# swiss-territorial-data-lab/proj-roadsurf

Hardware: AMD Instinct MI355X
Metric: tiles_per_sec_512x512x3 (higher is better)
Workload: dtype f16 hi + lo operand planes (22 significand bits, 3 MFMA products per product) / f32 accumulate; 1 GPU; Mask R-CNN R50-FPN inference, batch 16 of 512x512 3-band tiles per GPU (BASELINE configs[1]), 800x800 network input; seeded synthetic weights, saturated: 1000 proposals and 100 detections per tile; batch_per_gpu=16, lanes=2, lane_streams=independent, num_classes=2, weights=random

## Files before the change

include/rs_engine.h:

```cpp
#ifndef RS_ENGINE_H
#define RS_ENGINE_H

#include <stddef.h>
#include <stdint.h>

#ifdef __cplusplus
extern "C" {
#endif

#define RS_ABI_VERSION 1
#define RS_SPEC_MAX_LEVELS 5
#define RS_SPEC_MAX_ANCHORS 8
#define RS_NUM_PHASES 3
#define RS_MASK_SIDE 28

typedef struct rs_spec {
  int32_t struct_size;
  int32_t in_channels;
  int32_t flip_channels;
  float pixel_mean[4];
  float pixel_std[4];
  int32_t min_size_test;
  int32_t max_size_test;
  int32_t size_divisibility;
// ... 75 lines not shown
int rs_engine_set_profiling(rs_engine* e, int mode);
int rs_engine_stage_count(rs_engine* e);
int rs_engine_stage_info(rs_engine* e, int i, char* name_out, double* ms_total, int* calls, double* flops, double* bytes);
int rs_engine_saturation(rs_engine* e, int64_t* counts, int cap);
int rs_engine_stage_kernel(rs_engine* e, int i, char* name_out);
int rs_engine_stage_variant(rs_engine* e, int i);

int rs_engine_tensor(rs_engine* e, const char* name, void** dev_ptr, int* dtype, int* ndim, int64_t dims[5], int* halo);
int rs_engine_tensor_count(rs_engine* e);
int rs_engine_tensor_name(rs_engine* e, int i, char* name_out );

int rs_engine_net_shape(rs_engine* e, int* resized_h, int* resized_w, int* padded_h, int* padded_w);


int rs_op_conv2d(const void* in, const void* w, const float* bias, void* out, const void* residual,
                 const void* upsample_add, int n, int hi, int wi, int cin, int in_halo, int kh, int kw,
                 int stride, int pad, int cout, int kpad, int out_halo, int relu, int out_f32, int deconv2x,
                 int variant, int use_glds, void* stream);

int rs_op_bneck_tail(const void* t1, const void* w2, const float* b2, const void* w3p, const float* b3, const void* x, void* out,
                     const void* w1p, const float* b1, void* t1n, const void* x0, const void* wsc, int n, int h, int w, int width,
                     void* stream);

int rs_op_bneck_tail_split(const void* t1, int64_t t1_lo, const void* w2, const float* s2, const float* b2, const void* w3p, const float* s3,
                           const float* b3, const void* x, int64_t x_lo, void* out, int64_t out_lo, const void* w1p, const float* s1,
                           const float* b1, void* t1n, int64_t t1n_lo, const void* x0, int64_t x0_lo, int n, int h, int w, int width,
                           void* stream);

int rs_op_mask_overlap(const uint8_t* det_masks, int n_det, const uint8_t* label_masks, int n_labels, int h, int w, int32_t* inter,
                       int32_t* label_area, void* stream);
int rs_engine_label_overlap(rs_engine* e, int tile, const uint8_t* label_masks_dev, int n_labels, int32_t* inter_dev, int32_t* label_area_dev);

int rs_op_conv_variant(int m, int cin, int k, int cout, int cin2, int deconv2x, int out_f32, int* stages_out);

int rs_debug_set_conv_probe(void* buffer);

int rs_op_set_saturation_counter(void* dev_u64);

int rs_op_conv2d_split(const void* in, int64_t in_lo, const void* w, int64_t w_lo, const float* wscale, const float* bias, void* out, int64_t out_lo,
                       const void* residual, int64_t res_lo, const void* upsample_add, int64_t up_lo,
                       int n, int hi, int wi, int cin, int in_halo, int kh, int kw, int stride, int pad, int cout, int kpad,
                       int out_halo, int relu, int out_f32, int deconv2x, int variant, void* stream);

int rs_op_conv2d_dual(const void* in, const void* in2, const void* w, const float* bias, void* out,
                      int n, int hi, int wi, int cin, int in_halo, int kh, int kw, int stride, int pad,
                      int h2, int w2, int cin2, int in2_halo, int stride2,
                      int cout, int kpad, int out_halo, int relu, int variant, void* stream);

int rs_op_conv2d_dgrad(const void* dy, const void* w_t, void* dx, const void* res, const float* res32, const void* mask,
                       const void* down, int n, int hi, int wi, int cin, int ho, int wo, int cout, int kh, int kw, int stride,
                       int pad, int kpad, int halo, int variant, void* stream);

int rs_op_conv2d_wgrad(const void* dy, const void* in, float* grad, const float* scale, int n, int hi, int wi, int cin,
                       int in_halo, int kh, int kw, int stride, int pad, int cout, int kpad, int dy_halo, int splits,
                       void* stream);
int rs_op_conv2d_wgrad_f32(const void* dy, const void* in, float* grad, const float* scale, int n, int hi, int wi, int cin,
                       int in_halo, int kh, int kw, int stride, int pad, int cout, int kpad, int dy_halo, int splits,
                       void* stream);

int rs_op_nms(const float* boxes, const int32_t* counts, const uint8_t* valid, uint8_t* keep,
              int segments, int cap, float thresh, void* stream);

int rs_op_roi_align(const void* const feats[4], const int32_t heights[4], const int32_t widths[4],
                    const float scales[4], int nlevels, const float* rois, int n_rois, int rois_per_image,
                    int P, int out_halo, void* out, int32_t* levels_out, void* stream);

// ... 90 lines not shown
```

proj_roadsurf_amd/csrc/common.h:

```cpp
#pragma once
#include <hip/hip_runtime.h>
#include <stdint.h>
#include <stdio.h>

typedef _Float16 half_t;
typedef _Float16 half4 __attribute__((ext_vector_type(4)));
typedef _Float16 half8 __attribute__((ext_vector_type(8)));
typedef float f32x4 __attribute__((ext_vector_type(4)));

#define RS_OK 0
#define RS_ERR_ARG -1
#define RS_ERR_HIP -2
#define RS_ERR_BLOB -3
#define RS_ERR_UNSUPPORTED -4

void rs_set_error(const char* fmt, ...);

#define RS_HIP(expr)                                                                       \
  do {                                                                                     \
    hipError_t _e = (expr);                                                                \
    if (_e != hipSuccess) {                                                                \
      rs_set_error("%s:%d: %s -> %s", __FILE__, __LINE__, #expr, hipGetErrorString(_e));   \
      return RS_ERR_HIP;                                                                   \
    }                                                                                      \
// ... 220 lines not shown
int wgrad_splits(const WgradParams& p);
int launch_conv_wgrad(const WgradParams& p, hipStream_t stream);

struct PreprocParams {
  const uint8_t* tiles;
  half_t* out;
  const int* hb;
  const int* hk;
  const int* vb;
  const int* vk;
  int N, H, W, C;
  int new_h, new_w;
  int out_Hp, out_Wp;
  int ksh, ksv;
  int need_h, need_v;
  int flip;
  int out_f32;
  long long out_lo;
  float mean[4], stdv[4];
  unsigned long long* sat;
};
int launch_preprocess(const PreprocParams& p, hipStream_t s);
int launch_maxpool(const half_t* in, half_t* out, int N, int Hi, int Wi, int Ho, int Wo, int C, hipStream_t s);
int launch_subsample2(const half_t* in, half_t* out, int N, int Hi, int Wi, int Ho, int Wo, int C, hipStream_t s);
int launch_maxpool_f32(const float* in, float* out, int N, int Hi, int Wi, int Ho, int Wo, int C, hipStream_t s);
int launch_maxpool_split(const half_t* in, long long in_lo, half_t* out, long long out_lo, int N, int Hi, int Wi, int Ho, int Wo, int C, hipStream_t s);
int launch_subsample2_split(const half_t* in, long long in_lo, half_t* out, long long out_lo, int N, int Hi, int Wi, int Ho, int Wo, int C, hipStream_t s);
int launch_subsample2_f32(const float* in, float* out, int N, int Hi, int Wi, int Ho, int Wo, int C, hipStream_t s);
int launch_conv_f32(const ConvParams& p, hipStream_t stream, int force_valu = 0, int tile = 0);
int launch_conv_deep(const ConvParams& p, hipStream_t stream, int tile_px = 256);
int rs_device_cu_count();
bool conv_wreg_ok(const ConvParams& p);
int launch_conv_wreg(const ConvParams& p, hipStream_t stream, int waves = 0);
int launch_conv_deep_multi(const ConvParams& common, const ConvSeg* segs, const int* m_per_image, int nseg, int images, hipStream_t stream);
```

proj_roadsurf_amd/csrc/conv_igemm.hip:

```cpp
#include "common.h"

namespace {

template <int WPX, int WCH, int MI, int NJ>
struct Tile {
  static constexpr int NW = WPX * WCH;
  static constexpr int NT = NW * 64;
  static constexpr int BM = WPX * NJ * 16;
  static constexpr int BN = WCH * MI * 16;
  static constexpr int STAGE = (BM + BN) * 128;
  static constexpr int LDS = 2 * STAGE + 1024;
};

__device__ __forceinline__ void glds16(const half_t* g, char* lds_wave_base) {
  __builtin_amdgcn_global_load_lds((const __attribute__((address_space(1))) void*)g,
                                   (__attribute__((address_space(3))) void*)lds_wave_base, 16, 0, 0);
}

template <int WPX, int WCH, int MI, int NJ, bool SMALLC, bool GLDS, bool PERSIST, bool TRAIN = false, bool SPLIT = false>
__global__ __launch_bounds__(WPX* WCH * 64) void conv_igemm_kernel(const ConvParams p) {
  using T = Tile<WPX, WCH, MI, NJ>;
  constexpr int NW = T::NW, BM = T::BM, BN = T::BN;
  constexpr int PA = BM / (NW * 8);
  constexpr int PW = (BN + NW * 8 - 1) / (NW * 8);
// ... 465 lines not shown
  const void* k;
  if (p.split) {
    RS_CHECK(use_glds > 0 && !train && p.wscale, RS_ERR_UNSUPPORTED, "conv: the split-operand mode needs LDS-DMA staging, the row scales and no training epilogue");
    k = (const void*)conv_igemm_kernel<WPX, WCH, MI, NJ, SMALLC, true, false, false, true>;
  } else if (train) {
    RS_CHECK(use_glds && !SMALLC, RS_ERR_UNSUPPORTED, "conv: training epilogue options need LDS-DMA staging and Cin >= 64");
    if constexpr (!SMALLC) k = (const void*)conv_igemm_kernel<WPX, WCH, MI, NJ, false, true, false, true>;
    else k = nullptr;
  } else if constexpr (CAN_PERSIST) {
    k = persistent ? (const void*)conv_igemm_kernel<WPX, WCH, MI, NJ, SMALLC, true, true>
                   : (use_glds ? (const void*)conv_igemm_kernel<WPX, WCH, MI, NJ, SMALLC, true, false>
                               : (const void*)conv_igemm_kernel<WPX, WCH, MI, NJ, SMALLC, false, false>);
  } else {
    k = use_glds ? (const void*)conv_igemm_kernel<WPX, WCH, MI, NJ, SMALLC, true, false>
                 : (const void*)conv_igemm_kernel<WPX, WCH, MI, NJ, SMALLC, false, false>;
  }
  static bool attr[5] = {false, false, false, false, false};
  const int ai = p.split ? 4 : (train ? 3 : (persistent ? 2 : (use_glds ? 1 : 0)));
  if (!attr[ai]) {
    RS_HIP(hipFuncSetAttribute(k, hipFuncAttributeMaxDynamicSharedMemorySize, T::LDS));
    attr[ai] = true;
  }
  const unsigned grid = (persistent && !p.split) ? 256u * (unsigned)bpc : (unsigned)nblk;
  ConvParams pc = p;
  void* args[] = {&pc};
  RS_HIP(hipLaunchKernel(k, dim3(grid), dim3(T::NT), args, lds, stream));
  return RS_OK;
}

}

thread_local int g_last_conv_variant = -2;

int conv_choose_variant(ConvParams& p, int force_variant, int use_glds) {
  const RsDebug& D = rs_debug();
  const int nk2 = p.in2 ? (p.Cin2 >> 6) : 0;
  const bool smallc = p.Cin < 64;
  const int nk = (p.split ? 3 : 1) * (smallc ? (p.Kpad >> 6) : p.KH * p.KW * (p.Cin >> 6) + nk2);
  if (p.stages == 0) {
    const bool shallow = nk <= D.conv_single_stage_nk;
    if (D.conv_persist >= 1 && shallow && p.mode != 2 && !p.split) { p.stages = 2; p.persist = 2; }
    else { p.stages = shallow ? 1 : 2; p.persist = D.conv_persist >= 2 && p.mode != 2 ? -1 : 0; }
  }
  if (force_variant >= 0) return force_variant;
  const int rows = p.Cout * (p.mode != 0 ? 4 : 1);
  const int nkd = smallc ? 0 : nk;
  const long long tiles0 = (long long)cdiv(p.M, 128) * (rows / 128 > 0 ? rows / 128 : 1);
  const long long tiles4 = (long long)cdiv(p.M, 256) * (rows / 256 > 0 ? rows / 256 : 1);
  if (rows <= 16) return 2;
  if (!D.conv_tuned || p.mode != 0 || smallc) return rows % 128 == 0 ? 0 : 1;
  if (rows % 128 != 0) return 8;
  if (rows % 256 == 0 && nkd >= 8 && D.conv_deep && D.deep_tile_px && use_glds > 0 && !p.in2 && !p.m_count && !p.down && !p.res32 && !p.mask && p.out_stride <= 1) {
    const int ncu = 256;
    auto cost = [&](int nj) {
      const long long t = (long long)cdiv(p.M, 32 * nj) * (rows / 256);
      const long long r = t % ncu;
      const double rounds = (double)(t / ncu) + (r == 0 ? 0.0 : (nj == 8 && D.deep_tail && 2 * r <= ncu ? 0.75 : 1.0));
      return rounds * (nj + 15);
    };
    int best = 8;
    double cb = cost(8);
    for (int nj = 7; nj >= 5; --nj) {
      const long long t = (long long)cdiv(p.M, 32 * nj) * (rows / 256);
      if (4 * t >= 3 * ncu && cost(nj) < 0.95 * cb && cost(nj) < (best == 8 ? 1e30 : cost(best))) best = nj;
    }
    if (best != 8) return 10 + best;
  }
  if (p.split && rows % 256 == 0 && nkd >= 8 && tiles4 >= 64 && tiles4 < 240 && D.conv_deep && use_glds > 0 && !p.in2 && p.out_stride <= 1) return 12;
  if (p.in2 && rows % 256 == 0 && nkd >= 6) return tiles4 >= 600 ? 4 : (tiles0 < 1250 ? 7 : 0);
  if (rows % 256 == 0 && nkd >= 8 && tiles4 >= 240)
    return (D.conv_deep && use_glds > 0 && !p.in2 && p.out_stride <= 1) ? 12 : 4;
  if (D.conv_wreg && !p.split && use_glds > 0 && conv_wreg_ok(p) && (long long)cdiv(p.M, 32) * (p.Cout >> 8) * 5 >= 48ll * rs_device_cu_count()) return 22;
  if (rows % 256 == 0 && nkd <= 4 && p.M >= 40000) return D.conv_wide_px == 64 ? 10 : 14;
  if (nkd <= 4 || tiles0 < 1250) return 7;
  return 0;
}

int launch_conv(const ConvParams& p_in, hipStream_t stream, int force_variant, int use_glds) {
  if (use_glds < 0) {
    RS_CHECK(!p_in.in2, RS_ERR_UNSUPPORTED, "conv: the fp32 kernel has no second K source");
    g_last_conv_variant = -1;
    return launch_conv_f32(p_in, stream, use_glds == -2, force_variant);
  }
  ConvParams p = p_in;
  const int nk2 = p.in2 ? (p.Cin2 >> 6) : 0;
  const bool train_opts = p.down || p.res32 || p.mask || p.out_stride > 1;
  RS_CHECK(p.M > 0, RS_ERR_ARG, "conv: M=%d", p.M);
  RS_CHECK(p.Kpad % 64 == 0, RS_ERR_ARG, "conv: Kpad %d not a multiple of 64", p.Kpad);
  const bool smallc = p.Cin < 64;
  if (smallc) {
    RS_CHECK((p.Cin == 8 || p.Cin == 4) && p.koff != nullptr, RS_ERR_ARG, "conv: small-Cin path needs Cin 4 or 8 and a koff table");
  } else {
    RS_CHECK(p.Cin % 64 == 0, RS_ERR_ARG, "conv: Cin %d not a multiple of 64", p.Cin);
    RS_CHECK(p.KH * p.KW * p.Cin + nk2 * 64 <= p.Kpad, RS_ERR_ARG, "conv: K exceeds Kpad");
  }
  if (p.in2) RS_CHECK(!smallc && p.mode == 0 && p.Cin2 % 64 == 0 && p.Cin2 > 0 && p.stride2 >= 1, RS_ERR_ARG, "conv: bad second K source (Cin2 %d)", p.Cin2);
  const int rows = p.Cout * (p.mode != 0 ? 4 : 1);
  int v = conv_choose_variant(p, force_variant, use_glds);
  if (v == 22 && p.mode == 2 && !conv_wreg_ok(p)) v = 14;
  RS_CHECK(!(train_opts && (p.mode != 0 || (v == 12 && p.out_stride > 1) || (v >= 15 && v <= 20))), RS_ERR_UNSUPPORTED, "conv: training epilogue options need mode 0 (and no scatter on conv_deep)");
  if (v == 22 || v == 23 || v == 25 || v == 26) {
    RS_CHECK(conv_wreg_ok(p) && !train_opts, RS_ERR_UNSUPPORTED, "conv: variant %d takes 1x1 / Cin 256 / Cout %% 256 == 0 inference layers only", v);
    g_last_conv_variant = v;
    return launch_conv_wreg(p, stream, v == 23 ? 8 : (v == 25 ? 2 : (v == 26 ? 4 : 0)));
  }
  if (v == 12 || (v >= 15 && v <= 20)) {
    RS_CHECK(!p.in2, RS_ERR_UNSUPPORTED, "conv: variant %d has no second K source", v);
    g_last_conv_variant = v;
    return launch_conv_deep(p, stream, v == 12 ? 256 : (v <= 17 ? 160 + 32 * (v - 15) : 64 + 32 * (v - 18)));
  }
  RS_CHECK(!(p.mode != 0 && p.Cout % 128 != 0), RS_ERR_ARG, "deconv needs Cout %% 128 == 0");
  RS_CHECK(!(p.mode == 2 && !(p.dot_w && p.dot_cls && p.dot_slot && p.dot_out && (v == 0 || v == 10 || v == 14))), RS_ERR_ARG, "fused mask predictor needs its pointers and the 128x128, 64x256 or 128x256 tile");
  g_last_conv_variant = smallc ? 5 : v;
  if (smallc) {
    RS_CHECK(v == 1, RS_ERR_ARG, "conv: small-Cin path is built for the 256x64 tile only (Cout=%d)", p.Cout);
    if (rs_debug().stem_small_tile) return launch_variant<4, 1, 4, 2, true, false>(p, stream, use_glds);
    return launch_variant<4, 1, 4, 4, true, false>(p, stream, use_glds);
  }
  switch (v) {
    case 0:
      RS_CHECK(rows % 128 == 0, RS_ERR_ARG, "conv: variant 0 needs Cout %% 128 == 0");
      return launch_variant<2, 2, 4, 4, false, true>(p, stream, use_glds);
    case 1:
      RS_CHECK(rows % 64 == 0, RS_ERR_ARG, "conv: variant 1 needs Cout %% 64 == 0");
      return launch_variant<4, 1, 4, 4, false, true>(p, stream, use_glds);
    case 2:
      RS_CHECK(rows % 16 == 0 && p.out_f32, RS_ERR_ARG, "conv: variant 2 is the 16-channel-tile fp32-out head kernel");
      return launch_variant<4, 1, 1, 4, false, true>(p, stream, use_glds);
    case 7:
      RS_CHECK(rows % 128 == 0, RS_ERR_ARG, "conv: variant 7 needs Cout %% 128 == 0");
      return launch_variant<2, 2, 4, 2, false, false>(p, stream, use_glds);
    case 9:
      RS_CHECK(rows % 128 == 0, RS_ERR_ARG, "conv: variant 9 needs Cout %% 128 == 0");
      return launch_variant<2, 2, 4, 1, false, false>(p, stream, use_glds);
    case 10:
// ... 20 lines not shown
```

proj_roadsurf_amd/csrc/engine.hip:

```cpp
#include <stdarg.h>
#include <string.h>

#include <cmath>
#include <functional>
#include <map>
#include <set>
#include <string>
#include <vector>

#include "../../include/rs_engine.h"
#include "detect.h"
#include "train.h"

static thread_local char g_err[1024] = "";
static bool g_trainer_unfused_shortcut = false;

static RsDebug g_debug;
static bool g_debug_loaded = false;
void rs_debug_reload() {
  RsDebug d;
  auto rd = [](const char* name, int* v) { const char* e = getenv(name); if (e && *e) *v = atoi(e); };
  rd("RS_CONV_SINGLE_STAGE_NK", &d.conv_single_stage_nk); rd("RS_CONV_PERSIST", &d.conv_persist); rd("RS_CONV_TUNED", &d.conv_tuned);
  rd("RS_CONV_DEEP", &d.conv_deep); rd("RS_CONV_WIDE_PX", &d.conv_wide_px); rd("RS_CONV_WREG", &d.conv_wreg); rd("RS_WREG_DBG", &d.wreg_dbg); rd("RS_ROI_BWD_ATOMIC", &d.roi_bwd_atomic); rd("RS_WREG_WAVES", &d.wreg_waves); rd("RS_STEM_SMALL_TILE", &d.stem_small_tile); rd("RS_DEEP_DBG", &d.deep_dbg);
  rd("RS_DECONV_VARIANT", &d.deconv_variant); rd("RS_FUSE_MASK_PREDICTOR", &d.fuse_mask_predictor); rd("RS_SIDE_STREAM", &d.side_stream);
// ... 1003 lines not shown
    if ((rc = alloc((void**)&mask_probs, (size_t)R * RS_MASK_SIDE * RS_MASK_SIDE * 4))) return rc;
    reg("mask_probs", mask_probs, DT_F32, {NB, D, RS_MASK_SIDE, RS_MASK_SIDE}, 0);
    const BlobEntry* dw = findw("roi_heads.mask_head.deconv");
    const BlobEntry* db = find("roi_heads.mask_head.deconv.b");
    const BlobEntry* pw = find("roi_heads.mask_head.predictor.w");
    const BlobEntry* pb = find("roi_heads.mask_head.predictor.b");
    RS_CHECK(dw && db && wrows(dw) == 1024, RS_ERR_BLOB, "deconv weights missing / wrong rows");
    RS_CHECK(pw && pb && pw->dtype == DT_F32, RS_ERR_BLOB, "mask predictor weights missing");
    const bool fuse = f32 ? false : rs_debug().fuse_mask_predictor != 0;
    ConvParams dp;
    memset(&dp, 0, sizeof dp);
    if ((rc = set_split(&dp, "roi_heads.mask_head.deconv", dw, &curm, nullptr, nullptr, nullptr, nullptr))) return rc;
    dp.in = curm.p; dp.w = (const half_t*)dw->dev; dp.bias = (const float*)db->dev;
    dp.Ho = MR; dp.Wo = MR; dp.in_Hp = curm.Hp(); dp.in_Wp = curm.Wp(); dp.in_Cs = 256; dp.in_off = 1; dp.stride = 1; dp.KH = dp.KW = 1;
    dp.Cin = 256; dp.Kpad = (int)dw->dims[1]; dp.Cout = 256; dp.out_Hp = 2 * MR; dp.out_Wp = 2 * MR; dp.out_Cs = 256; dp.out_pad = 0; dp.relu = 1;
    dp.m_count = det_total; dp.m_mul = MR * MR;
    const int per_roi = MR * MR;
    if (fuse) {
      dp.mode = 2; dp.out = nullptr;
      dp.dot_w = (const float*)pw->dev; dp.dot_cls = det_classes; dp.dot_slot = slot_list; dp.dot_out = mask_probs;
      dp.dot_k = (int)pw->dims[0];
      const int glds = use_glds, Dc = D;
      const bool sp = split;
      float* probs = mask_probs;
      const size_t zero_per_tile = (size_t)D * RS_MASK_SIDE * RS_MASK_SIDE * 4;
      Stage st;
      st.name = "mask.deconv_predict";
      st.flops_per_image = 2.0 * D * per_roi * 256 * 1024 + 2.0 * D * RS_MASK_SIDE * RS_MASK_SIDE * 256;
      st.bytes_per_image = (double)D * per_roi * 256 * 2 * (split ? 2 : 1) + (double)D * RS_MASK_SIDE * RS_MASK_SIDE * 4;
      st.fn = [dp, per_roi, Dc, glds, probs, zero_per_tile, sp](int n, hipStream_t s) mutable {
        RS_HIP(hipMemsetAsync(probs, 0, zero_per_tile * n, s));
        dp.M = n * Dc * per_roi;
        const int dv = rs_debug().deconv_variant;
        return launch_conv(dp, s, (dv == 22 && (sp || !(rs_debug().conv_wreg && glds > 0))) ? 14 : dv, glds);
      };
      stages.push_back(st);
      MaskPredictParams mp;
      mp.f32 = 0;
      mp.in = nullptr; mp.w = nullptr; mp.b = (const float*)pb->dev; mp.slot_list = slot_list; mp.det_classes = det_classes;
      mp.n_entries = det_total; mp.out = mask_probs; mp.S = RS_MASK_SIDE;
      Stage st2;
      st2.name = "mask.bias_sigmoid";
      st2.fn = [mp, Dc](int n, hipStream_t s) { return launch_mask_sigmoid(mp, n * Dc, s); };
      stages.push_back(st2);
    } else {
      Act dec;
      if ((rc = new_act(&dec, "mask_deconv", R, 2 * MR, 2 * MR, 256, 0))) return rc;
      dp.mode = 1; dp.out = dec.p; dp.out_lo = dec.lo;
      {
        const int glds = use_glds, Dc = D;
        Stage st;
        st.name = "mask.deconv";
        st.flops_per_image = 2.0 * D * per_roi * 256 * 1024;
        st.bytes_per_image = (double)D * per_roi * 256 * 2 * 5;
        dp.sat = sat_slot();
        st.fn = [dp, per_roi, Dc, glds](int n, hipStream_t s) mutable { dp.M = n * Dc * per_roi; return launch_conv(dp, s, -1, glds); };
        stages.push_back(st);
      }
      MaskPredictParams mp;
      mp.in = dec.p; mp.w = (const float*)pw->dev; mp.b = (const float*)pb->dev; mp.slot_list = slot_list; mp.det_classes = det_classes;
      mp.n_entries = det_total; mp.out = mask_probs; mp.S = RS_MASK_SIDE; mp.f32 = f32 ? 1 : (split ? 2 : 0); mp.in_lo = dec.lo;
      Stage st;
      st.name = "mask.predict_sigmoid";
      st.bytes_per_image = (double)D * RS_MASK_SIDE * RS_MASK_SIDE * (256 * 2 + 4);
      const int Dc = D;
      st.fn = [mp, Dc](int n, hipStream_t s) { return launch_mask_predict(mp, n * Dc, s); };
      stages.push_back(st);
// ... 440 lines not shown
int rs_engine_stage_count(rs_engine* e) { return e ? (int)e->stages.size() : 0; }
int rs_engine_saturation(rs_engine* e, int64_t* counts, int cap) {
  RS_CHECK(e && (counts || cap <= 0), RS_ERR_ARG, "null argument");
  const int n = (int)e->stages.size();
  for (int i = 0; i < n && i < cap; ++i) counts[i] = i < (int)e->h_sat.size() ? e->h_sat[i] : 0;
  return n;
}
int rs_engine_stage_info(rs_engine* e, int i, char* name_out, double* ms_total, int* calls, double* flops, double* bytes) {
  RS_CHECK(e && i >= 0 && i < (int)e->stages.size(), RS_ERR_ARG, "stage index");
  if (e->ev_used) { int rc = e->resolve_profile(); if (rc) return rc; }
  const Stage& s = e->stages[i];
  if (name_out) { strncpy(name_out, s.name.c_str(), 95); name_out[95] = 0; }
  if (ms_total) *ms_total = s.ms_total;
  if (calls) *calls = s.calls;
  if (flops) *flops = s.last_flops;
  if (bytes) *bytes = s.last_bytes;
  return RS_OK;
}

int rs_engine_stage_kernel(rs_engine* e, int i, char* name_out) {
  RS_CHECK(e && i >= 0 && i < (int)e->stages.size() && name_out, RS_ERR_ARG, "stage index");
  static const char* names[] = {"conv_igemm_kernel<2,2,4,4> 128x128", "conv_igemm_kernel<4,1,4,4> 256x64", "conv_igemm_kernel<4,1,1,4> 256x16 f32-out",
                                "conv_igemm_kernel<4,2,4,4> 256x128", "conv_igemm_kernel<2,4,4,8> 256x256", "conv_igemm_kernel<4,1,4,4,smallC> 256x64 stem",
                                "(retired)",
                                "conv_igemm_kernel<2,2,4,2> 64x128", "conv_igemm_kernel<4,1,4,2> 128x64", "conv_igemm_kernel<2,2,4,1> 32x128",
                                "conv_igemm_kernel<2,4,4,2> 64x256", "(retired)",
                                "conv_deep_kernel 256x256 (3 activation + 2 weight LDS stages)",
                                "bneck_tail_kernel 128 px (conv2 + conv3 + next conv1 chained through registers)",
                                "conv_igemm_kernel<2,4,4,4> 128x256",
                                "conv_deep_kernel 160x256", "conv_deep_kernel 192x256", "conv_deep_kernel 224x256",
                                "conv_deep_kernel 64x256", "conv_deep_kernel 96x256", "conv_deep_kernel 128x256",
                                "stem_pool_kernel (conv 7x7 s2 + ReLU + max-pool 3x3 s2, 8x8 pooled pixels per workgroup)",
                                "conv1x1_wreg_kernel 32 px x 256 ch (persistent, weights in registers, operand tiles by LDS-DMA, two workgroups per CU)",
                                "bneck_tail_split_kernel 128 px (conv2 + conv3 + next conv1 chained through registers)"};
  const int v = e->stages[i].variant;
  const char* s = v == -1 ? "conv_f32_mfma_kernel" : (v >= 0 && v <= 23 ? names[v] : "");
  if (e->split && v >= 0 && v <= 23) {
    snprintf(name_out, 96, "%.62s [split: hi+lo planes, 3 MFMA blocks]", s);
    return RS_OK;
  }
  strncpy(name_out, s, 95);
  name_out[95] = 0;
  return RS_OK;
}

int rs_engine_stage_variant(rs_engine* e, int i) {
  if (!e || i < 0 || i >= (int)e->stages.size()) return -2;
  return e->stages[i].variant;
}

int rs_op_conv_variant(int m, int cin, int k, int cout, int cin2, int deconv2x, int out_f32, int* stages_out) {
  ConvParams p;
  memset(&p, 0, sizeof p);
  p.M = m; p.Cin = cin; p.KH = p.KW = k; p.Cout = cout; p.mode = deconv2x ? 1 : 0; p.out_f32 = out_f32;
  p.stride = 1; p.in_Cs = cin; p.out_Cs = cout;
  p.Kpad = (k * k * (cin < 64 ? 8 : cin) + cin2 + 63) / 64 * 64;
  if (cin < 64 && k == 7) p.Kpad = 256;
  static const half_t dummy = (half_t)0;
  if (cin2 > 0) { p.in2 = &dummy; p.Cin2 = cin2; }
  const int v = conv_choose_variant(p, -1, 1);
  if (stages_out) *stages_out = p.stages;
  return cin < 64 ? 5 : v;
}

int rs_engine_tensor(rs_engine* e, const char* name, void** dev_ptr, int* dtype, int* ndim, int64_t dims[5], int* halo) {
  RS_CHECK(e && name, RS_ERR_ARG, "null argument");
  for (const TensorInfo& t : e->tensors) {
    if (t.name == name) {
      if (dev_ptr) *dev_ptr = t.p;
      if (dtype) *dtype = t.dtype;
      if (ndim) *ndim = t.ndim;
      if (dims) for (int i = 0; i < 5; ++i) dims[i] = t.dims[i];
      if (halo) *halo = t.halo;
      return RS_OK;
    }
  }
  rs_set_error("no tensor named %s", name);
  return RS_ERR_ARG;
}
int rs_engine_tensor_count(rs_engine* e) { return e ? (int)e->tensors.size() : 0; }
int rs_engine_tensor_name(rs_engine* e, int i, char* name_out) {
  RS_CHECK(e && i >= 0 && i < (int)e->tensors.size() && name_out, RS_ERR_ARG, "tensor index");
  strncpy(name_out, e->tensors[i].name.c_str(), 95);
  name_out[95] = 0;
  return RS_OK;
}

int rs_engine_net_shape(rs_engine* e, int* rh, int* rw, int* ph, int* pw) {
  RS_CHECK(e, RS_ERR_ARG, "null engine");
  if (rh) *rh = e->net_h;
  if (rw) *rw = e->net_w;
  if (ph) *ph = e->pad_h;
  if (pw) *pw = e->pad_w;
  return RS_OK;
}
// ... 312 lines not shown
```

proj_roadsurf_amd/engine.py:

```python
from __future__ import annotations

import ctypes as C
import weakref
import math
import os
import time
from typing import Any, Dict, Iterator, List, Optional, Sequence, Tuple

import numpy as np

from .spec import EngineSpec
from .weights import pack_weights

_LIB: Optional[C.CDLL] = None
LIB_PATH = os.environ.get("RS_ENGINE_LIB") or os.path.join(os.path.dirname(os.path.abspath(__file__)), "librs_engine.so")
MAX_LEVELS, MAX_ANCHORS, MASK_SIDE = 5, 8, 28
DT_NP = {1: np.float16, 2: np.float32, 3: np.int32, 4: np.uint8, 5: np.float16}
DT_SPLIT16 = 5


class RsError(RuntimeError):
    pass


# ... 58 lines not shown
                      "(hipcc, gfx950). There is no CPU fallback for the detection path.")
    lib = C.CDLL(p)
    vp, i32, f32p, i32p, u8p = C.c_void_p, C.c_int, C.POINTER(C.c_float), C.POINTER(C.c_int32), C.POINTER(C.c_uint8)
    lib.rs_last_error.restype = C.c_char_p
    lib.rs_abi_version.restype = i32
    lib.rs_engine_create.argtypes = [C.POINTER(RsSpec), vp, C.c_size_t, i32, i32, i32, i32, i32, vp, C.POINTER(vp)]
    lib.rs_engine_destroy.argtypes = [vp]
    lib.rs_engine_destroy.restype = None
    lib.rs_engine_infer.argtypes = [vp, vp, i32, C.POINTER(RsDets)]
    lib.rs_engine_infer_device.argtypes = [vp, vp, i32]
    lib.rs_engine_infer_phase.argtypes = [vp, vp, i32, i32]
    lib.rs_engine_sync.argtypes = [vp]
    lib.rs_host_alloc.argtypes = [C.c_size_t]
    lib.rs_host_alloc.restype = vp
    lib.rs_host_free.argtypes = [vp]
    lib.rs_host_free.restype = None
    lib.rs_engine_upload_async.argtypes = [vp, vp, i32]
    lib.rs_engine_fetch_async.argtypes = [vp, i32, C.POINTER(RsDets)]
    lib.rs_engine_fetch_wait.argtypes = [vp]
    lib.rs_engine_fetch_crops_async.argtypes = [vp, i32, C.POINTER(RsDets), C.POINTER(RsMaskCrops)]
    lib.rs_engine_fetch_crops_wait.argtypes = [vp, C.POINTER(RsMaskCrops)]
    lib.rs_engine_fetch.argtypes = [vp, i32, C.POINTER(RsDets)]
    lib.rs_engine_stream.argtypes = [vp]
    lib.rs_engine_stream.restype = vp
    lib.rs_engine_set_profiling.argtypes = [vp, i32]
    lib.rs_debug_run_stages_matching.argtypes = [vp, C.c_char_p, i32]
    lib.rs_engine_stage_count.argtypes = [vp]
    lib.rs_engine_saturation.argtypes = [vp, C.POINTER(C.c_int64), i32]
    lib.rs_op_set_saturation_counter.argtypes = [vp]
    lib.rs_engine_stage_info.argtypes = [vp, i32, C.c_char_p, C.POINTER(C.c_double), i32p, C.POINTER(C.c_double), C.POINTER(C.c_double)]
    lib.rs_engine_stage_kernel.argtypes = [vp, i32, C.c_char_p]
    lib.rs_engine_stage_variant.argtypes = [vp, i32]
    lib.rs_op_conv_variant.argtypes = [i32] * 7 + [i32p]
    lib.rs_engine_tensor.argtypes = [vp, C.c_char_p, C.POINTER(vp), i32p, i32p, C.POINTER(C.c_int64), i32p]
    lib.rs_engine_tensor_count.argtypes = [vp]
    lib.rs_engine_tensor_name.argtypes = [vp, i32, C.c_char_p]
    lib.rs_engine_net_shape.argtypes = [vp, i32p, i32p, i32p, i32p]
    lib.rs_op_conv2d.argtypes = [vp, vp, vp, vp, vp, vp] + [i32] * 17 + [vp]
    lib.rs_op_bneck_tail.argtypes = [vp] * 12 + [i32, i32, i32, i32, vp]
    lib.rs_op_conv2d_dual.argtypes = [vp, vp, vp, vp, vp] + [i32] * 19 + [vp]
    i64 = C.c_int64
    lib.rs_op_conv2d_split.argtypes = [vp, i64, vp, i64, vp, vp, vp, i64, vp, i64, vp, i64] + [i32] * 16 + [vp]
    lib.rs_op_bneck_tail_split.argtypes = [vp, i64, vp, vp, vp, vp, vp, vp, vp, i64, vp, i64, vp, vp, vp, vp, i64, vp, i64, i32, i32, i32, i32, vp]
    lib.rs_op_conv2d_dgrad.argtypes = [vp] * 7 + [i32] * 14 + [vp]
    lib.rs_op_conv2d_wgrad.argtypes = [vp, vp, vp, vp] + [i32] * 13 + [vp]
    lib.rs_op_nms.argtypes = [vp, vp, vp, vp, i32, i32, C.c_float, vp]
    lib.rs_op_roi_align.argtypes = [C.POINTER(vp), i32p, i32p, f32p, i32, vp, i32, i32, i32, i32, vp, vp, vp]
    lib.rs_op_roi_align_bwd.argtypes = [C.POINTER(vp), i32p, i32p, f32p, i32, vp, i32, i32, i32, i32, vp, vp]
    f32 = C.c_float
    lib.rs_op_match.argtypes = [vp, i32, vp, vp, vp, vp, vp, vp, i32, i32, i32, f32, f32, i32, i32, i32, i32, vp]
    lib.rs_op_subsample.argtypes = [vp, vp, vp, i32, i32, i32, f32, i32, i32, C.c_uint32, vp]
    lib.rs_op_rpn_loss.argtypes = [vp] * 6 + [i32] * 6 + [f32, f32, vp]
    lib.rs_op_box_loss.argtypes = [vp] * 6 + [i32, i32, i32, f32, f32p, f32, vp]
    lib.rs_op_mask_loss.argtypes = [vp] * 5 + [i32, i32, i32, f32, vp]
    lib.rs_op_sgd_momentum.argtypes = [vp, vp, vp, C.c_int64, f32, f32, f32, f32, i32, vp]
    lib.rs_op_fold_weights.argtypes = [vp] * 4 + [i32] * 6 + [vp]
    lib.rs_resize_shape.argtypes = [i32, i32, i32, i32, i32p, i32p]
    lib.rs_resize_shape.restype = None
    lib.rs_resize_coeffs.argtypes = [i32, i32, i32p, i32p]
    i64p, f64p = C.POINTER(C.c_int64), C.POINTER(C.c_double)
    lib.rs_vectorize_masks.argtypes = [vp, i32, i32, i32, C.c_double, i32]
    lib.rs_vectorize_masks.restype = vp
    lib.rs_vec_counts.argtypes = [vp, i64p, i64p, i64p, i64p]
    lib.rs_vec_counts.restype = None
    lib.rs_vec_copy.argtypes = [vp, i32p, i32p, i32p, f64p]
    lib.rs_vec_free.argtypes = [vp]
# ... 1035 lines not shown
```

Baseline: 938.8 tiles/s.

## Add persistent weights-in-registers 1x1 conv kernel for split hi/lo operands

Adds a new persistent 1x1 convolution kernel for the split-precision path. It keeps hi and lo weight planes in registers, streams the hi/lo activation tiles (and residual or upsample operands) into an LDS ring with LDS-DMA, and runs three MFMA products per step. It is routed in for large split-mode 1x1 layers with Cin 256, including the mask deconv predictor. Before this, split mode fell back to the generic tiled kernels. The cost is high register and LDS use at one workgroup per CU, and a walk-length threshold decides which layers take the new path.

```diff
diff --git a/include/rs_engine.h b/include/rs_engine.h
--- a/include/rs_engine.h
+++ b/include/rs_engine.h
@@ -131,6 +131,7 @@
 int rs_engine_label_overlap(rs_engine* e, int tile, const uint8_t* label_masks_dev, int n_labels, int32_t* inter_dev, int32_t* label_area_dev);
 
 int rs_op_conv_variant(int m, int cin, int k, int cout, int cin2, int deconv2x, int out_f32, int* stages_out);
+int rs_op_conv_variant_split(int m, int cin, int k, int cout, int cin2, int deconv2x, int out_f32, int* stages_out);
 
 int rs_debug_set_conv_probe(void* buffer);
 
diff --git a/proj_roadsurf_amd/csrc/common.h b/proj_roadsurf_amd/csrc/common.h
--- a/proj_roadsurf_amd/csrc/common.h
+++ b/proj_roadsurf_amd/csrc/common.h
@@ -276,4 +276,6 @@
 int rs_device_cu_count();
 bool conv_wreg_ok(const ConvParams& p);
 int launch_conv_wreg(const ConvParams& p, hipStream_t stream, int waves = 0);
+bool conv_wreg_split_ok(const ConvParams& p);
+int launch_conv_wreg_split(const ConvParams& p, hipStream_t stream);
 int launch_conv_deep_multi(const ConvParams& common, const ConvSeg* segs, const int* m_per_image, int nseg, int images, hipStream_t stream);
diff --git a/proj_roadsurf_amd/csrc/conv_igemm.hip b/proj_roadsurf_amd/csrc/conv_igemm.hip
--- a/proj_roadsurf_amd/csrc/conv_igemm.hip
+++ b/proj_roadsurf_amd/csrc/conv_igemm.hip
@@ -521,6 +521,7 @@
 
 thread_local int g_last_conv_variant = -2;
 
+constexpr int SPLIT_WREG_WALK = 10;
 int conv_choose_variant(ConvParams& p, int force_variant, int use_glds) {
   const RsDebug& D = rs_debug();
   const int nk2 = p.in2 ? (p.Cin2 >> 6) : 0;
@@ -539,6 +540,7 @@
   if (rows <= 16) return 2;
   if (!D.conv_tuned || p.mode != 0 || smallc) return rows % 128 == 0 ? 0 : 1;
   if (rows % 128 != 0) return 8;
+  if (D.conv_wreg && p.split && use_glds > 0 && conv_wreg_ok(p) && (long long)cdiv(p.M, 32) * (p.Cout >> 8) >= (long long)SPLIT_WREG_WALK * rs_device_cu_count()) return 24;
   if (rows % 256 == 0 && nkd >= 8 && D.conv_deep && D.deep_tile_px && use_glds > 0 && !p.in2 && !p.m_count && !p.down && !p.res32 && !p.mask && p.out_stride <= 1) {
     const int ncu = 256;
     auto cost = [&](int nj) {
@@ -586,10 +588,15 @@
   if (p.in2) RS_CHECK(!smallc && p.mode == 0 && p.Cin2 % 64 == 0 && p.Cin2 > 0 && p.stride2 >= 1, RS_ERR_ARG, "conv: bad second K source (Cin2 %d)", p.Cin2);
   const int rows = p.Cout * (p.mode != 0 ? 4 : 1);
   int v = conv_choose_variant(p, force_variant, use_glds);
-  if (v == 22 && p.mode == 2 && !conv_wreg_ok(p)) v = 14;
+  if (((v == 22 && !conv_wreg_ok(p)) || (v == 24 && !conv_wreg_split_ok(p))) && p.mode == 2) v = 14;
   RS_CHECK(!(train_opts && (p.mode != 0 || (v == 12 && p.out_stride > 1) || (v >= 15 && v <= 20))), RS_ERR_UNSUPPORTED, "conv: training epilogue options need mode 0 (and no scatter on conv_deep)");
+  if (v == 24) {
+    RS_CHECK(conv_wreg_split_ok(p) && !train_opts, RS_ERR_UNSUPPORTED, "conv: variant 24 takes split-operand 1x1 / Cin 256 / Cout %% 256 == 0 inference layers only");
+    g_last_conv_variant = v;
+    return launch_conv_wreg_split(p, stream);
+  }
   if (v == 22 || v == 23 || v == 25 || v == 26) {
-    RS_CHECK(conv_wreg_ok(p) && !train_opts, RS_ERR_UNSUPPORTED, "conv: variant %d takes 1x1 / Cin 256 / Cout %% 256 == 0 inference layers only", v);
+    RS_CHECK(conv_wreg_ok(p) && !train_opts && !p.split, RS_ERR_UNSUPPORTED, "conv: variant %d takes fp16 1x1 / Cin 256 / Cout %% 256 == 0 inference layers only", v);
     g_last_conv_variant = v;
     return launch_conv_wreg(p, stream, v == 23 ? 8 : (v == 25 ? 2 : (v == 26 ? 4 : 0)));
   }
diff --git a/proj_roadsurf_amd/csrc/conv_wreg_split.hip b/proj_roadsurf_amd/csrc/conv_wreg_split.hip
--- /dev/null
+++ b/proj_roadsurf_amd/csrc/conv_wreg_split.hip
@@ -0,0 +1,380 @@
+#include "common.h"
+
+namespace {
+
+constexpr int MI = 4;
+
+__device__ __forceinline__ void glds16(const half_t* g, char* lds_wave_base) {
+  __builtin_amdgcn_global_load_lds((const __attribute__((address_space(1))) void*)g,
+                                   (__attribute__((address_space(3))) void*)lds_wave_base, 16, 0, 0);
+}
+
+struct Pix { int x, y, n; };
+__device__ __forceinline__ Pix pix_add(int x0, int y0, int n0, int rx, int ry, int rn, int Wo, int Ho) {
+  int x = x0 + rx;
+  const int cx = x >= Wo;
+  x -= cx ? Wo : 0;
+  int y = y0 + ry + cx;
+  const int cy = y >= Ho;
+  y -= cy ? Ho : 0;
+  return Pix{x, y, n0 + rn + cy};
+}
+
+template <int EPI, int BM, int NA>
+__global__ __launch_bounds__(256, 1) void conv1x1_wreg_split_kernel(const ConvParams p, const int dbg) {
+  constexpr int SLICE = BM * 128;
+  constexpr int ACT = 4 * SLICE;
+  constexpr int NJ = BM / 16;
+  constexpr int PASSES = BM / 32;
+  constexpr bool OPND = EPI == 1 || EPI == 2;
+  constexpr int TILE = 2 * ACT;
+  constexpr int D = NA - 1;
+  constexpr int OPB = NA * TILE;
+  static_assert(D == 2 || (D == 3 && !OPND), "two or three tiles ahead; the operand ring holds two");
+  constexpr int OPS = (OPND ? 16 : 8) * PASSES;
+  constexpr int STS = 4 * NJ;
+  static_assert((D - 1) * OPS + D * STS < 64, "the counted wait must fit vmcnt");
+  extern __shared__ __attribute__((aligned(16))) char smem[];
+  const int tid = threadIdx.x, lane = tid & 63;
+  const int wch = __builtin_amdgcn_readfirstlane(tid >> 6);
+  int Mv = p.M;
+  if (p.m_count) { const long long mc = (long long)(*p.m_count) * p.m_mul; if (mc < Mv) Mv = (int)mc; }
+  const int M = Mv, Wo = p.Wo, Ho = p.Ho;
+  const int tiles_m = (M + BM - 1) / BM;
+  const int groups = EPI == 3 ? 4 : p.Cout >> 8;
+  int L;
+  {
+    const int G = gridDim.x, qn = G >> 3, r = G & 7, x = blockIdx.x & 7;
+    L = (x < r ? x * (qn + 1) : r * (qn + 1) + (x - r) * qn) + (blockIdx.x >> 3);
+  }
+  const int grp = L % groups, first = L / groups, step = gridDim.x / groups;
+  const int ntl = first < tiles_m ? (tiles_m - 1 - first) / step + 1 : 0;
+  if (ntl == 0) return;
+  const int n0 = grp * 256;
+  const int fi = lane & 15, fq = lane >> 4, fkey = lane & 7;
+  const int lrow = lane >> 3, lchk = lane & 7;
+
+  const int HW = Ho * Wo;
+  int tx, ty, tn;
+  { const int m = first * BM; tn = m / HW; const int r = m - tn * HW; ty = r / Wo; tx = r - ty * Wo; }
+  int dx, dy, dn;
+  { const int m = step * BM; dn = m / HW; const int r = m - dn * HW; dy = r / Wo; dx = r - dy * Wo; }
+  int ex = tx, ey = ty, en = tn;
+  int irx[PASSES], iry[PASSES], irn[PASSES];
+#pragma unroll
+  for (int ps = 0; ps < PASSES; ++ps) {
+    const int r = ps * 32 + wch * 8 + lrow;
+    irn[ps] = r / HW; const int q = r - irn[ps] * HW; iry[ps] = q / Wo; irx[ps] = q - iry[ps] * Wo;
+  }
+  int orx[NJ], ory[NJ], orn[NJ];
+#pragma unroll
+  for (int j = 0; j < NJ; ++j) {
+    const int r = j * 16 + fi;
+    orn[j] = r / HW; const int q = r - orn[j] * HW; ory[j] = q / Wo; orx[j] = q - ory[j] * Wo;
+  }
+  const int c0_off = (fq ^ fkey) * 16, c1_off = ((4 + fq) ^ fkey) * 16;
+  const int ec0 = ((2 * fq) ^ fkey) * 16, ec1 = ((2 * fq + 1) ^ fkey) * 16;
+  const int sw8 = (lchk ^ lrow) * 8;
+  const int crow = n0 + wch * 64 + fq * 16;
+
+  auto issue_tile = [&](int m0, int aslot, int oslot) {
+    if (dbg & 4) return;
+    char* base = smem + aslot * TILE;
+    char* obase = smem + OPB + oslot * TILE;
+#pragma unroll
+    for (int ps = 0; ps < PASSES; ++ps) {
+      const int r = ps * 32 + wch * 8 + lrow;
+      Pix q = pix_add(tx, ty, tn, irx[ps], iry[ps], irn[ps], Wo, Ho);
+      if (m0 + r >= M) q = Pix{tx, ty, tn};
+      const half_t* src = p.in + ((long long)(q.n * p.in_Hp + q.y + p.in_off) * p.in_Wp + q.x + p.in_off) * p.in_Cs + sw8;
+      char* dst = base + (ps * 32 + wch * 8) * 128;
+      char* odst = obase + (ps * 32 + wch * 8) * 128;
+#pragma unroll
+      for (int s = 0; s < 4; ++s) glds16(src + s * 64, dst + s * SLICE);
+#pragma unroll
+      for (int s = 0; s < 4; ++s) glds16(src + p.in_lo + s * 64, dst + ACT + s * SLICE);
+      if (OPND) {
+        const half_t* es;
+        long long elo;
+        if (EPI == 1) { es = p.res + ((long long)(q.n * p.out_Hp + q.y + p.out_pad) * p.out_Wp + q.x + p.out_pad) * p.out_Cs + n0; elo = p.res_lo; }
+        else { es = p.up + ((long long)(q.n * p.up_Hp + (q.y >> 1) + p.up_pad) * p.up_Wp + (q.x >> 1) + p.up_pad) * p.up_Cs + n0; elo = p.up_lo; }
+        es += sw8;
+#pragma unroll
+        for (int s = 0; s < 4; ++s) glds16(es + s * 64, odst + s * SLICE);
+#pragma unroll
+        for (int s = 0; s < 4; ++s) glds16(es + elo + s * 64, odst + ACT + s * SLICE);
+      }
+    }
+    const Pix nx = pix_add(tx, ty, tn, dx, dy, dn, Wo, Ho);
+    tx = nx.x; ty = nx.y; tn = nx.n;
+  };
+
+#pragma unroll
+  for (int t = 0; t < D; ++t)
+    if (t < ntl) issue_tile((first + t * step) * BM, t, t & 1);
+
+  half8 wh[8][MI], wl[8][MI];
+#pragma unroll
+  for (int i = 0; i < MI; ++i) {
+    const int row = n0 + wch * 64 + (fi >> 2) * 16 + i * 4 + (fi & 3);
+    const half_t* wr = p.w + (long long)row * p.Kpad + fq * 8;
+#pragma unroll
+    for (int t = 0; t < 8; ++t) {
+      wh[t][i] = *(const half8*)(wr + t * 32);
+      wl[t][i] = *(const half8*)(wr + p.w_lo + t * 32);
+    }
+  }
+  float bias[16], wsc[16];
+#pragma unroll
+  for (int i = 0; i < MI; ++i) {
+    const f32x4 b4 = *(const f32x4*)(p.bias + crow + i * 4);
+    const f32x4 s4 = *(const f32x4*)(p.wscale + crow + i * 4);
+#pragma unroll
+    for (int r = 0; r < 4; ++r) { bias[i * 4 + r] = b4[r]; wsc[i * 4 + r] = s4[r]; }
+  }
+  float* const red = (float*)(smem + OPB);
+  float* const wcls = red + 256;
+  int* const ent_slot = (int*)(wcls + (EPI == 3 ? p.dot_k : 0) * 256);
+  const int n_ent = EPI == 3 ? p.M / (Ho * Wo) : 0;
+  int* const ent_cls = ent_slot + n_ent;
+  if constexpr (EPI == 3) {
+    for (int i = tid; i < p.dot_k * 256; i += 256) wcls[i] = p.dot_w[i];
+    const int n_valid = (M + Ho * Wo - 1) / (Ho * Wo);
+    for (int e = tid; e < n_ent; e += 256) {
+      int sl = 0, cl = 0;
+      if (e < n_valid) { sl = p.dot_slot[e]; cl = p.dot_cls[sl]; }
+      ent_slot[e] = sl; ent_cls[e] = cl;
+    }
+    __syncthreads();
+  }
+  asm volatile("s_waitcnt vmcnt(0)" ::: "memory");
+  int x_off[NJ], e_off[NJ];
+#pragma unroll
+  for (int j = 0; j < NJ; ++j) {
+    x_off[j] = (j * 16 + fi) * 128;
+    e_off[j] = OPB + wch * SLICE + (j * 16 + fi) * 128;
+  }
+
+  int as = 0, is = D;
+  for (int k = 0; k < ntl; ++k) {
+    if (k >= D) {
+      constexpr int ST = EPI == 3 ? NJ : STS;
+      const int st = (EPI == 3 && wch != 0) ? 0 : D * ST;
+      const int left = ntl - 1 - k;
+      const int rem = left < D - 1 ? left : D - 1;
+      if (st == 0) {
+        if (rem == 0) asm volatile("s_waitcnt vmcnt(0)" ::: "memory");
+        else if (rem == 1) asm volatile("s_waitcnt vmcnt(%0)" ::"n"(OPS) : "memory");
+        else if constexpr (D >= 3) asm volatile("s_waitcnt vmcnt(%0)" ::"n"(2 * OPS) : "memory");
+      } else {
+        if (rem == 0) asm volatile("s_waitcnt vmcnt(%0)" ::"n"(D * ST) : "memory");
+        else if (rem == 1) asm volatile("s_waitcnt vmcnt(%0)" ::"n"(D * ST + OPS) : "memory");
+        else if constexpr (D >= 3) asm volatile("s_waitcnt vmcnt(%0)" ::"n"(D * ST + 2 * OPS) : "memory");
+      }
+    }
+    __builtin_amdgcn_s_barrier();
+    __builtin_amdgcn_sched_barrier(0);
+    half8 e0h[NJ], e1h[NJ], e0l[NJ], e1l[NJ];
+    if (OPND) {
+      const char* ob = smem + (k & 1) * TILE;
+#pragma unroll
+      for (int j = 0; j < NJ; ++j) {
+        e0h[j] = *(const half8*)(ob + e_off[j] + ec0);
+        e1h[j] = *(const half8*)(ob + e_off[j] + ec1);
+        e0l[j] = *(const half8*)(ob + ACT + e_off[j] + ec0);
+        e1l[j] = *(const half8*)(ob + ACT + e_off[j] + ec1);
+      }
+      asm volatile("s_waitcnt lgkmcnt(0)" ::: "memory");
+      __builtin_amdgcn_s_barrier();
+      __builtin_amdgcn_sched_barrier(0);
+    }
+    if (k + D < ntl) issue_tile((first + (k + D) * step) * BM, is, k & 1);
+    __builtin_amdgcn_sched_barrier(0);
+    f32x4 acc[MI][NJ];
+#pragma unroll
+    for (int i = 0; i < MI; ++i)
+#pragma unroll
+      for (int j = 0; j < NJ; ++j) acc[i][j] = f32x4{0.f, 0.f, 0.f, 0.f};
+    const char* sb = smem + as * TILE;
+    as = as + 1 == NA ? 0 : as + 1;
+    is = is + 1 == NA ? 0 : is + 1;
+    half8 xh[2][NJ], xl[2][NJ];
+    auto frags = [&](int t) {
+      const int co = (t >> 1) * SLICE + ((t & 1) ? c1_off : c0_off);
+#pragma unroll
+      for (int j = 0; j < NJ; ++j) { xh[t & 1][j] = *(const half8*)(sb + x_off[j] + co); xl[t & 1][j] = *(const half8*)(sb + ACT + x_off[j] + co); }
+    };
+    if (!(dbg & 2)) frags(0);
+#pragma unroll
+    for (int t = 0; t < 8; ++t) {
+      if (dbg & 2) break;
+      if (t + 1 < 8) frags(t + 1);
+      __builtin_amdgcn_sched_barrier(0);
+#pragma unroll
+      for (int i = 0; i < MI; ++i)
+#pragma unroll
+        for (int j = 0; j < NJ; ++j) acc[i][j] = __builtin_amdgcn_mfma_f32_16x16x32_f16(wh[t][i], xl[t & 1][j], acc[i][j], 0, 0, 0);
+#pragma unroll
+      for (int i = 0; i < MI; ++i)
+#pragma unroll
+        for (int j = 0; j < NJ; ++j) acc[i][j] = __builtin_amdgcn_mfma_f32_16x16x32_f16(wh[t][i], xh[t & 1][j], acc[i][j], 0, 0, 0);
+#pragma unroll
+      for (int i = 0; i < MI; ++i)
+#pragma unroll
+        for (int j = 0; j < NJ; ++j) acc[i][j] = __builtin_amdgcn_mfma_f32_16x16x32_f16(wl[t][i], xh[t & 1][j], acc[i][j], 0, 0, 0);
+      __builtin_amdgcn_sched_barrier(0);
+    }
+    const int m0 = (first + k * step) * BM;
+    if ((dbg & 1) && acc[0][0][0] != 12345.f) continue;
+    if constexpr (EPI == 3) {
+      float dotp[NJ];
+      long long dot_idx[NJ];
+      const int g = grp, cb = wch * 64 + fq * 16;
+#pragma unroll
+      for (int j = 0; j < NJ; ++j) {
+        dotp[j] = 0.f; dot_idx[j] = -1;
+        const int m = m0 + j * 16 + fi;
+        if (m >= M) continue;
+        const Pix q = pix_add(ex, ey, en, orx[j], ory[j], orn[j], Wo, Ho);
+        const int oy = 2 * q.y + (g >> 1), ox = 2 * q.x + (g & 1);
+        float v[16];
+#pragma unroll
+        for (int i = 0; i < MI; ++i)
+#pragma unroll
+          for (int r = 0; r < 4; ++r) v[i * 4 + r] = acc[i][j][r] * wsc[i * 4 + r] + bias[i * 4 + r];
+        if (p.relu) {
+#pragma unroll
+          for (int e = 0; e < 16; ++e) v[e] = v[e] > 0.f ? v[e] : 0.f;
+        }
+        const int slot = ent_slot[q.n];
+        const float* wv = wcls + ent_cls[q.n] * 256 + cb;
+        float sdot = 0.f;
+#pragma unroll
+        for (int i = 0; i < MI; ++i) {
+          const f32x4 w4 = *(const f32x4*)(wv + i * 4);
+#pragma unroll
+          for (int r = 0; r < 4; ++r) sdot += v[i * 4 + r] * w4[r];
+        }
+        dotp[j] = sdot;
+        dot_idx[j] = (long long)slot * (4 * Ho * Wo) + (long long)oy * (2 * Wo) + ox;
+      }
+#pragma unroll
+      for (int j = 0; j < NJ; ++j) {
+        float v0 = dotp[j];
+        v0 += __shfl_xor(v0, 16);
+        v0 += __shfl_xor(v0, 32);
+        dotp[j] = v0;
+        if (wch > 0 && fq == 0) red[((wch - 1) * NJ + j) * 16 + fi] = v0;
+      }
+      asm volatile("s_waitcnt lgkmcnt(0)" ::: "memory");
+      __builtin_amdgcn_s_barrier();
+      __builtin_amdgcn_sched_barrier(0);
+      if (wch == 0 && fq == 0) {
+#pragma unroll
+        for (int j = 0; j < NJ; ++j) {
+          float v0 = dotp[j];
+#pragma unroll
+          for (int c = 1; c < 4; ++c) v0 += red[((c - 1) * NJ + j) * 16 + fi];
+          if (dot_idx[j] >= 0) atomicAdd(p.dot_out + dot_idx[j], v0);
+        }
+      }
+      { const Pix nx = pix_add(ex, ey, en, dx, dy, dn, Wo, Ho); ex = nx.x; ey = nx.y; en = nx.n; }
+      continue;
+    }
+#pragma unroll
+    for (int j = 0; j < NJ; ++j) {
+      const int m = m0 + j * 16 + fi;
+      if (m >= M) continue;
+      const Pix q = pix_add(ex, ey, en, orx[j], ory[j], orn[j], Wo, Ho);
+      const long long opix = (long long)(q.n * p.out_Hp + q.y + p.out_pad) * p.out_Wp + q.x + p.out_pad;
+      float v[16];
+#pragma unroll
+      for (int i = 0; i < MI; ++i)
+#pragma unroll
+        for (int r = 0; r < 4; ++r) v[i * 4 + r] = acc[i][j][r] * wsc[i * 4 + r] + bias[i * 4 + r];
+      if (OPND) {
+#pragma unroll
+        for (int r = 0; r < 8; ++r) {
+          v[r] += (float)e0h[j][r] + (float)e0l[j][r];
+          v[8 + r] += (float)e1h[j][r] + (float)e1l[j][r];
+        }
+      }
+      if (p.relu) {
+#pragma unroll
+        for (int e = 0; e < 16; ++e) v[e] = v[e] > 0.f ? v[e] : 0.f;
+      }
+      half_t* op = (half_t*)p.out + opix * p.out_Cs + crow;
+      float scr = 0.f;
+#pragma unroll
+      for (int i = 0; i < 2; ++i) {
+        half8 h, l;
+#pragma unroll
+        for (int r = 0; r < 8; ++r) {
+          float f = v[i * 8 + r];
+          f = f > 65504.f ? 65504.f : (f < -65504.f ? -65504.f : f);
+          scr += __builtin_fabsf(f);
+          h[r] = (half_t)f;
+          l[r] = (half_t)(f - (float)h[r]);
+        }
+        *(half8*)(op + i * 8) = h;
+        *(half8*)(op + p.out_lo + i * 8) = l;
+      }
+      if (!(scr < 65504.f)) {
+        unsigned c = 0;
+#pragma unroll
+        for (int e = 0; e < 16; ++e) c += rs_sat_bad(v[e]);
+        rs_sat_flush(p.sat, c);
+        asm volatile("s_waitcnt vmcnt(0)" ::: "memory");
+      }
+    }
+    { const Pix nx = pix_add(ex, ey, en, dx, dy, dn, Wo, Ho); ex = nx.x; ey = nx.y; en = nx.n; }
+  }
+}
+
+constexpr int SPLIT_EPI3_TABLES = 31 * 1024;
+int epi3_tables(const ConvParams& p) { return 1024 + p.dot_k * 1024 + (p.M / (p.Ho * p.Wo)) * 8; }
+
+int no_scratch(const void* kernel, const char* what) {
+  hipFuncAttributes a;
+  RS_HIP(hipFuncGetAttributes(&a, kernel));
+  RS_CHECK(a.localSizeBytes == 0, RS_ERR_UNSUPPORTED, "%s was built with %zu bytes of scratch per thread (rebuild with the documented toolchain)", what,
+           (size_t)a.localSizeBytes);
+  return RS_OK;
+}
+
+template <int EPI, int BM, int NA>
+int launch_wreg_split(const ConvParams& p, hipStream_t stream) {
+  constexpr int ring = (NA + ((EPI == 1 || EPI == 2) ? 2 : 0)) * 2 * 4 * BM * 128;
+  constexpr int lds_max = ring + (EPI == 3 ? SPLIT_EPI3_TABLES : 0);
+  static_assert(lds_max <= 160 * 1024, "ring beyond the LDS");
+  static bool done = false;
+  if (!done) {
+    RS_HIP(hipFuncSetAttribute((const void*)conv1x1_wreg_split_kernel<EPI, BM, NA>, hipFuncAttributeMaxDynamicSharedMemorySize, lds_max));
+    { int rc = no_scratch((const void*)conv1x1_wreg_split_kernel<EPI, BM, NA>, "conv1x1_wreg_split_kernel"); if (rc) return rc; }
+    done = true;
+  }
+  int lds = ring;
+  if (EPI == 3) lds += epi3_tables(p);
+  const int groups = EPI == 3 ? 4 : p.Cout >> 8, tiles_m = cdiv(p.M, BM);
+  int per_group = rs_device_cu_count() / groups;
+  if (per_group < 1) per_group = 1;
+  if (per_group > tiles_m) per_group = tiles_m;
+  hipLaunchKernelGGL((conv1x1_wreg_split_kernel<EPI, BM, NA>), dim3((unsigned)(per_group * groups)), dim3(256), lds, stream, p,
+                     EPI == 3 ? rs_debug().wreg_dbg >> 4 : rs_debug().wreg_dbg & 15);
+  RS_HIP(hipGetLastError());
+  return RS_OK;
+}
+
+}
+
+bool conv_wreg_split_ok(const ConvParams& p) {
+  return conv_wreg_ok(p) && p.split && p.wscale && (p.mode != 2 || epi3_tables(p) <= SPLIT_EPI3_TABLES);
+}
+
+int launch_conv_wreg_split(const ConvParams& p, hipStream_t stream) {
+  RS_CHECK(conv_wreg_split_ok(p) && p.M > 0, RS_ERR_ARG, "conv_wreg_split: shape outside the kernel's rules");
+  if (p.mode == 2) return launch_wreg_split<3, 32, 4>(p, stream);
+  if (p.res) return launch_wreg_split<1, 32, 3>(p, stream);
+  if (p.up) return launch_wreg_split<2, 32, 3>(p, stream);
+  return launch_wreg_split<0, 32, 4>(p, stream);
+}
diff --git a/proj_roadsurf_amd/csrc/engine.hip b/proj_roadsurf_amd/csrc/engine.hip
--- a/proj_roadsurf_amd/csrc/engine.hip
+++ b/proj_roadsurf_amd/csrc/engine.hip
@@ -1059,7 +1059,8 @@
         RS_HIP(hipMemsetAsync(probs, 0, zero_per_tile * n, s));
         dp.M = n * Dc * per_roi;
         const int dv = rs_debug().deconv_variant;
-        return launch_conv(dp, s, (dv == 22 && (sp || !(rs_debug().conv_wreg && glds > 0))) ? 14 : dv, glds);
+        const bool wreg = rs_debug().conv_wreg && glds > 0;
+        return launch_conv(dp, s, dv == 22 ? (!wreg ? 14 : (sp ? 24 : 22)) : dv, glds);
       };
       stages.push_back(st);
       MaskPredictParams mp;
@@ -1566,10 +1567,11 @@
                                 "conv_deep_kernel 64x256", "conv_deep_kernel 96x256", "conv_deep_kernel 128x256",
                                 "stem_pool_kernel (conv 7x7 s2 + ReLU + max-pool 3x3 s2, 8x8 pooled pixels per workgroup)",
                                 "conv1x1_wreg_kernel 32 px x 256 ch (persistent, weights in registers, operand tiles by LDS-DMA, two workgroups per CU)",
-                                "bneck_tail_split_kernel 128 px (conv2 + conv3 + next conv1 chained through registers)"};
+                                "bneck_tail_split_kernel 128 px (conv2 + conv3 + next conv1 chained through registers)",
+                                "conv1x1_wreg_split_kernel 32 px x 256 ch (persistent, weights in registers)"};
   const int v = e->stages[i].variant;
-  const char* s = v == -1 ? "conv_f32_mfma_kernel" : (v >= 0 && v <= 23 ? names[v] : "");
-  if (e->split && v >= 0 && v <= 23) {
+  const char* s = v == -1 ? "conv_f32_mfma_kernel" : (v >= 0 && v <= 24 ? names[v] : "");
+  if (e->split && v >= 0 && v <= 24) {
     snprintf(name_out, 96, "%.62s [split: hi+lo planes, 3 MFMA blocks]", s);
     return RS_OK;
   }
@@ -1583,9 +1585,10 @@
   return e->stages[i].variant;
 }
 
-int rs_op_conv_variant(int m, int cin, int k, int cout, int cin2, int deconv2x, int out_f32, int* stages_out) {
+static int op_conv_variant(int m, int cin, int k, int cout, int cin2, int deconv2x, int out_f32, int* stages_out, int split) {
   ConvParams p;
   memset(&p, 0, sizeof p);
+  p.split = split;
   p.M = m; p.Cin = cin; p.KH = p.KW = k; p.Cout = cout; p.mode = deconv2x ? 1 : 0; p.out_f32 = out_f32;
   p.stride = 1; p.in_Cs = cin; p.out_Cs = cout;
   p.Kpad = (k * k * (cin < 64 ? 8 : cin) + cin2 + 63) / 64 * 64;
@@ -1595,6 +1598,12 @@
   const int v = conv_choose_variant(p, -1, 1);
   if (stages_out) *stages_out = p.stages;
   return cin < 64 ? 5 : v;
+}
+int rs_op_conv_variant(int m, int cin, int k, int cout, int cin2, int deconv2x, int out_f32, int* stages_out) {
+  return op_conv_variant(m, cin, k, cout, cin2, deconv2x, out_f32, stages_out, 0);
+}
+int rs_op_conv_variant_split(int m, int cin, int k, int cout, int cin2, int deconv2x, int out_f32, int* stages_out) {
+  return op_conv_variant(m, cin, k, cout, cin2, deconv2x, out_f32, stages_out, 1);
 }
 
 int rs_engine_tensor(rs_engine* e, const char* name, void** dev_ptr, int* dtype, int* ndim, int64_t dims[5], int* halo) {
diff --git a/proj_roadsurf_amd/engine.py b/proj_roadsurf_amd/engine.py
--- a/proj_roadsurf_amd/engine.py
+++ b/proj_roadsurf_amd/engine.py
@@ -114,6 +114,7 @@
     lib.rs_engine_stage_kernel.argtypes = [vp, i32, C.c_char_p]
     lib.rs_engine_stage_variant.argtypes = [vp, i32]
     lib.rs_op_conv_variant.argtypes = [i32] * 7 + [i32p]
+    lib.rs_op_conv_variant_split.argtypes = [i32] * 7 + [i32p]
     lib.rs_engine_tensor.argtypes = [vp, C.c_char_p, C.POINTER(vp), i32p, i32p, C.POINTER(C.c_int64), i32p]
     lib.rs_engine_tensor_count.argtypes = [vp]
     lib.rs_engine_tensor_name.argtypes = [vp, i32, C.c_char_p]
```

After: 938.6 tiles/s. Within noise of the previous version (-0.0%).
